# PatrykChrabaszcz/HpBandSter

Hardware: AMD Instinct MI355X
Metric: candidate KDE evals/sec (cand×obs pairs) at D=32, 1/2/4/8 MI355X; % VALU peak (higher is better)
Workload: dtype f16 MFMA coarse pre-screen (1 product per dim, rigorous bound), f32 accumulate, f64 re-score

## Files before the change

hpbandster_amd/csrc/hbx_acquire.h:

```cpp
#pragma once
#include "hbx_score.h"

struct KdePairRef {
  int32_t D;
  const void* params_good;
  const float* table_good;
  const double* X_good;
  const int64_t* rows_good;
  int32_t variant_good;
  const void* params_bad;
  const float* table_bad;
  const double* X_bad;
  const int64_t* rows_bad;
  int32_t variant_bad, dc_pad, du_pad;
  int64_t nmax;
  const KdeParams* Pg() const { return (const KdeParams*)params_good; }
  const KdeParams* Pb() const { return (const KdeParams*)params_bad; }
};

struct WsLayout {
  size_t res, U, count, flags, segcnt, segnear, best, key, first1, rescue, est_l, est_g, lo, list, near, exact_l,
      exact_g, part, total;
  size_t stage, seeds, surv, lpart;
  int32_t list_cap;
};
#define STAGED_LIST_CAP 4096
WsLayout ws_layout(int64_t Nc, int64_t nmax, int64_t B = 1);

struct AcqWs {
  AcqResult* res;
  uint32_t* U;
  int32_t *count, *flags, *segcnt, *segnear;
  uint64_t *best, *key;
  int32_t *first1, *rescue;
  KdeEst *el, *eg;
  float* lo;
  int32_t *list, *near;
  double *exact_l, *exact_g, *part;
  uint32_t* stage;
  int32_t *seeds, *surv;
  KdeEst* lpart;
  int32_t list_cap;
  AcqWs(void* workspace, const WsLayout& w) {
    char* ws = (char*)workspace;
    res = (AcqResult*)(ws + w.res);
    U = (uint32_t*)(ws + w.U);
    count = (int32_t*)(ws + w.count);
    flags = (int32_t*)(ws + w.flags);
    segcnt = (int32_t*)(ws + w.segcnt);
    segnear = (int32_t*)(ws + w.segnear);
    best = (uint64_t*)(ws + w.best);
    key = (uint64_t*)(ws + w.key);
    first1 = (int32_t*)(ws + w.first1);
    rescue = (int32_t*)(ws + w.rescue);
    el = (KdeEst*)(ws + w.est_l);
    eg = (KdeEst*)(ws + w.est_g);
    lo = (float*)(ws + w.lo);
    list = (int32_t*)(ws + w.list);
    near = (int32_t*)(ws + w.near);
    exact_l = (double*)(ws + w.exact_l);
    exact_g = (double*)(ws + w.exact_g);
    part = (double*)(ws + w.part);
    stage = (uint32_t*)(ws + w.stage);
    seeds = (int32_t*)(ws + w.seeds);
    surv = (int32_t*)(ws + w.surv);
    lpart = (KdeEst*)(ws + w.lpart);
    list_cap = w.list_cap;
  }
  KdePairArgs::AcqInitPtrs init() const { return {U, count, flags, first1, res}; }
};

struct AcqPlan {
  ScoreFns fg, fb;
  bool exact_only;
};
const KdePairRef* acq_pair(const char* who, const void* pair);
int acq_check(const char* who, const KdePairRef& p, const double* cand, int64_t Nc, const void* workspace);
int acq_plan(const KdePairRef& p, bool fast, AcqPlan* plan);
int acq_score(const AcqPlan& plan, const KdePairRef& p, const AcqWs& a, const ScoreRequest& rq, int64_t batch_B,
              ScoreResult* out);
#ifndef HBX_STAGED_MIN_PAIRS
#define HBX_STAGED_MIN_PAIRS 1e9
#endif
bool acq_staged_supported(const AcqPlan& plan);
int acq_score_staged(const AcqPlan& plan, const KdePairRef& p, const double* cand, int64_t Nc, const AcqWs& a,
                     hipEvent_t* ev, hipStream_t s);
int acq_exact_only_init(int64_t Nc, uint32_t seg, const AcqWs& a, hipStream_t s);
#define EXACT_SCAN_MAX 1024
int acq_exact(const KdePairRef& p, const double* cand, int64_t Nc, const AcqWs& a, bool scan, bool combine,
              hipStream_t s);
```

hpbandster_amd/csrc/hbx_common.h:

```cpp
#pragma once

#include <hip/hip_runtime.h>
#include <stdint.h>
#include <stdlib.h>

#define HBX_MAX_D 256
#define HBX_WAVE 64

#include "hbx.h"

int hbx_fail(int code, const char* fmt, ...);

#define HBX_HIP(call)                                                                 \
  do {                                                                                \
    hipError_t _e = (call);                                                           \
    if (_e != hipSuccess)                                                             \
      return hbx_fail(HBX_ERR_HIP, "%s failed: %s (%s:%d)", #call, hipGetErrorString(_e), \
                      __FILE__, __LINE__);                                            \
  } while (0)

#define HBX_LAUNCH_CHECK()                                                            \
  do {                                                                                \
    hipError_t _e = hipGetLastError();                                                \
    if (_e != hipSuccess)                                                             \
      return hbx_fail(HBX_ERR_HIP, "kernel launch failed: %s (%s:%d)",               \
                      hipGetErrorString(_e), __FILE__, __LINE__);                    \
  } while (0)

static inline bool hbx_switch_on(const char* name) {
  const char* e = getenv(name);
  return !(e && atoi(e) == 0);
}
static inline int hbx_staged_mode() {
  const char* e = getenv("HBX_STAGED");
  if (!e) return 1;
  const int v = atoi(e);
  return v == 0 ? 0 : v == 2 ? 2 : 1;
}

struct KdeParams {
  int32_t n;
  int32_t D;
  int32_t dc;
  int32_t du;
  int32_t nconst;
  int32_t nan_all;
  int32_t has_neg;
  int32_t unsupported;
  int32_t stride;
  int32_t dc_pad;
  int32_t du_pad;
  int32_t exact_only;
  double log_norm;
  double m0_log2;
  double lb_sum;
  double prod_bw_c;
  float cmax;
  float sum_abs_delta;
  float cmax2;
  int32_t pad1;
  int32_t kc;
  int32_t hmode;
  int32_t nsc;
  int32_t chunk_floats;
  int32_t oh_total;
  int32_t coarse_off;
  int32_t coarse_chunk_floats;
  const double* X;
  const int64_t* rows;
  int32_t oh_dim[64];
  int32_t oh_level[64];
  int32_t oh_col[64];
  double oh_val[64];
  int32_t oh_start[64];
  int32_t cat_maxcode[HBX_MAX_D];
  int32_t cont_dim[HBX_MAX_D];
  double cont_scale[HBX_MAX_D];
  double center[HBX_MAX_D];
  float xmax[HBX_MAX_D];
  int32_t cat_dim[HBX_MAX_D];
  float cat_delta[HBX_MAX_D];
  float cat_negf[HBX_MAX_D];
  int32_t const_dim[HBX_MAX_D];
  double const_level[HBX_MAX_D];
  int32_t vartype[HBX_MAX_D];
  int32_t nlev[HBX_MAX_D];
  double bw[HBX_MAX_D];
};

#define HBX_PARAM_STAGE ((sizeof(KdeParams) + 255) & ~(size_t)255)
#define HBX_COLSTATS_OFF (HBX_PARAM_STAGE + 8 * HBX_MAX_D + 4 * HBX_MAX_D + 64)
#define HBX_PARAM_BYTES (HBX_COLSTATS_OFF + 8 * HBX_MAX_D + 4 * HBX_MAX_D)
struct ColStats {
  double mean[HBX_MAX_D];
  int32_t maxcode[HBX_MAX_D];
};

struct KdeEst {
  float lpos;
  float lneg;
  float err;
  float pad;
};

struct AcqResult {
  int64_t index;
  double score;
  float rel;
  int32_t flags;
  int32_t shortlist;
  int32_t near;
  double pdf_l;
  double pdf_g;
};

__device__ __forceinline__ void hbx_publish_store(uint32_t* dst, uint32_t v) {
  __hip_atomic_store(dst, v, __ATOMIC_RELAXED, __HIP_MEMORY_SCOPE_SYSTEM);
}
__device__ __forceinline__ void hbx_publish_store64(uint64_t* dst, uint64_t v) {
  __hip_atomic_store(dst, v, __ATOMIC_RELAXED, __HIP_MEMORY_SCOPE_SYSTEM);
}
__device__ __forceinline__ void hbx_publish_done(int32_t* done, int32_t seq) {
  __asm__ volatile("s_waitcnt vmcnt(0)" ::: "memory");
  __hip_atomic_store(done, seq, __ATOMIC_RELAXED, __HIP_MEMORY_SCOPE_SYSTEM);
}

__device__ __forceinline__ uint32_t hbx_f2ord(float f) {
  uint32_t u = __float_as_uint(f);
  return (u & 0x80000000u) ? ~u : (u | 0x80000000u);
}
__device__ __forceinline__ float hbx_ord2f(uint32_t u) {
  return __uint_as_float((u & 0x80000000u) ? (u & 0x7fffffffu) : ~u);
}

__device__ __forceinline__ uint64_t hbx_d2ord(double d) {
  if (d != d) return ~0ull;
  if (d == 0.0) d = 0.0;
  uint64_t u = (uint64_t)__double_as_longlong(d);
  return (u & 0x8000000000000000ull) ? ~u : (u | 0x8000000000000000ull);
}

template <typename Op>
__device__ __forceinline__ uint32_t wave_reduce_dpp(uint32_t v, Op op) {
  v = op(v, (uint32_t)__builtin_amdgcn_update_dpp(0, (int)v, 0xb1, 0xf, 0xf, false));
  v = op(v, (uint32_t)__builtin_amdgcn_update_dpp(0, (int)v, 0x4e, 0xf, 0xf, false));
  v = op(v, (uint32_t)__builtin_amdgcn_update_dpp(0, (int)v, 0x141, 0xf, 0xf, false));
  v = op(v, (uint32_t)__builtin_amdgcn_update_dpp(0, (int)v, 0x140, 0xf, 0xf, false));
  return op(op((uint32_t)__builtin_amdgcn_readlane((int)v, 0), (uint32_t)__builtin_amdgcn_readlane((int)v, 16)),
            op((uint32_t)__builtin_amdgcn_readlane((int)v, 32), (uint32_t)__builtin_amdgcn_readlane((int)v, 48)));
}
struct OpAdd { __device__ uint32_t operator()(uint32_t a, uint32_t b) const { return a + b; } };
struct OpAnd { __device__ uint32_t operator()(uint32_t a, uint32_t b) const { return a & b; } };
struct OpOr { __device__ uint32_t operator()(uint32_t a, uint32_t b) const { return a | b; } };
struct OpMax { __device__ uint32_t operator()(uint32_t a, uint32_t b) const { return a > b ? a : b; } };
```

hpbandster_amd/csrc/hbx_kde.hip:

```cpp
#include "hbx_acquire.h"

#include <string.h>

#include <new>

#include "hbx_acq_impl.h"
#include "hbx_host.h"
#include "hbx_pairwise.h"
#include "hbx_rescue_impl.h"


__global__ void acq_init_kernel(uint32_t* U, int32_t* count, int32_t* flags, int32_t* first1, AcqResult* res) {
  if (threadIdx.x == 0 && blockIdx.x == 0) acq_init_state(U, count, flags, first1, res);
}

__global__ void acq_init_batch_kernel(int64_t B, uint32_t* __restrict__ U, int32_t* __restrict__ flags,
                                      int32_t* __restrict__ segcnt, uint64_t* __restrict__ best,
                                      uint64_t* __restrict__ key, int32_t* __restrict__ first1,
                                      int32_t* __restrict__ count, int32_t* __restrict__ segnear) {
  const int64_t b = (int64_t)blockIdx.x * blockDim.x + threadIdx.x;
  if (b == 0) *count = 0;
  if (b < B) {
    U[b] = hbx_f2ord(INFINITY);
    flags[b] = 0;
// ... 412 lines not shown
}

__global__ __launch_bounds__(256) void kde_exact_logs_kernel(const int32_t* __restrict__ list,
                                                             const int32_t* __restrict__ count,
                                                             const double* __restrict__ exact_l,
                                                             const double* __restrict__ exact_g,
                                                             float* __restrict__ logl, float* __restrict__ logg) {
  const int p = blockIdx.x * 256 + threadIdx.x;
  if (p >= *count) return;
  const int i = list[p];
  if (logl) logl[i] = (float)log(exact_l[p]);
  if (logg) logg[i] = (float)log(exact_g[p]);
}


WsLayout ws_layout(int64_t Nc, int64_t nmax, int64_t B) {
  WsLayout w;
  size_t o = 0;
  auto take = [&](size_t bytes) {
    size_t r = o;
    o += (bytes + 255) & ~(size_t)255;
    return r;
  };
  w.res = take(sizeof(AcqResult));
  w.count = take(4);
  w.U = take(4 * B);
  w.flags = take(4 * B);
  w.segcnt = take(4 * B);
  w.segnear = take(4 * B);
  w.best = take(8 * B);
  w.key = take(8 * B);
  w.first1 = take(4 * B);
  w.rescue = take(4);
  const int sp = obs_splits((unsigned)((Nc + 511) / 512), nmax, true);
  const int64_t cap16 = 16 * Nc < 196608 ? 16 * Nc : 196608;
  const int64_t nest = Nc * sp > cap16 ? Nc * sp : cap16;
  w.est_l = take(sizeof(KdeEst) * nest);
  w.est_g = take(sizeof(KdeEst) * nest);
  w.lo = take(4 * Nc);
  w.list = take(4 * Nc);
  w.near = take(4 * Nc);
  w.exact_l = take(8 * Nc);
  w.exact_g = take(8 * Nc);
  w.part = take(8 * (size_t)2 * EXACT_SPLIT_CAP * PW_SPLIT_UNITS * ((nmax + PW_BUF - 1) / PW_BUF));
  static_assert(sizeof(AcqResult) + 4 * HBX_ST_WORDS <= 256, "the state words fit the result slot's padding");
  w.stage = w.res + sizeof(AcqResult);
  const int64_t tiles = (Nc + 511) / 512;
  w.list_cap = (int32_t)(512 * (tiles < 1 ? 1 : tiles > STAGED_LIST_CAP / 512 ? STAGED_LIST_CAP / 512 : tiles));
  w.seeds = take(4 * (size_t)w.list_cap);
  w.surv = take(4 * Nc);
  w.lpart = take(sizeof(KdeEst) * (size_t)OBS_SPLIT_MAX * w.list_cap);
  w.total = o;
  return w;
}

int acq_check(const char* who, const KdePairRef& p, const double* cand, int64_t Nc, const void* workspace) {
  if ((!cand && Nc > 0) || !p.params_good || !p.table_good || !p.X_good || !p.rows_good || !p.params_bad ||
      !p.table_bad || !p.X_bad || !p.rows_bad || !workspace)
    return hbx_fail(HBX_ERR_ARG, "%s: null pointer", who);
  if (Nc < 0 || Nc > INT32_MAX) return hbx_fail(HBX_ERR_ARG, "Nc=%lld out of range", (long long)Nc);
  return HBX_OK;
}

const KdePairRef* acq_pair(const char* who, const void* pair) {
  if (!pair) hbx_fail(HBX_ERR_ARG, "%s: null pair", who);
  return (const KdePairRef*)pair;
}

int acq_plan(const KdePairRef& p, bool fast, AcqPlan* plan) {
  plan->exact_only = KdeVariant::decode(p.variant_good).exact_only || KdeVariant::decode(p.variant_bad).exact_only;
  plan->fg = pick_logpdf(p.dc_pad, p.du_pad, p.variant_good, fast);
  plan->fb = pick_logpdf(p.dc_pad, p.du_pad, p.variant_bad, fast);
  if (!plan->exact_only && (!plan->fg.main || !plan->fb.main))
    return hbx_fail(HBX_ERR_UNSUPPORTED, "no kernel for dc_pad=%d du_pad=%d", p.dc_pad, p.du_pad);
  return HBX_OK;
}

int acq_score(const AcqPlan& plan, const KdePairRef& p, const AcqWs& a, const ScoreRequest& rq, int64_t batch_B,
              ScoreResult* out) {
  *out = ScoreResult{};
  const hipStream_t s = rq.s;
  const bool scored = rq.Nc > 0 && !plan.exact_only;
  if (scored) {
    const int rc = launch_score2({plan.fg, p.params_good, p.table_good, a.el},
                                 {plan.fb, p.params_bad, p.table_bad, a.eg}, rq, out);
    if (rc) return rc;
  }
  if (batch_B) {
    hipLaunchKernelGGL(acq_init_batch_kernel, dim3((unsigned)((batch_B + 255) / 256)), dim3(256), 0, s, batch_B, a.U,
                       a.flags, a.segcnt, a.best, a.key, a.first1, a.count, a.segnear);
    HBX_LAUNCH_CHECK();
  } else if (!out->inited) {
    hipLaunchKernelGGL(acq_init_kernel, dim3(1), dim3(64), 0, s, a.U, a.count, a.flags, a.first1, a.res);
    HBX_LAUNCH_CHECK();
  }
  if (scored && (out->nsplit[0] > 1 || out->nsplit[1] > 1)) {
    hipLaunchKernelGGL(kde_merge_splits_kernel, dim3((unsigned)((2 * rq.Nc + 255) / 256)), dim3(256), 0, s, a.el,
                       a.eg, rq.Nc, out->nsplit[0], out->nsplit[1]);
    HBX_LAUNCH_CHECK();
  }
  return HBX_OK;
}

int acq_exact_only_init(int64_t Nc, uint32_t seg, const AcqWs& a, hipStream_t s) {
  hipLaunchKernelGGL(kde_exact_only_init_kernel, dim3((unsigned)((Nc + 255) / 256)), dim3(256), 0, s, Nc, seg, a.el,
                     a.eg, a.lo, a.flags);
  HBX_LAUNCH_CHECK();
  return HBX_OK;
}

struct AcqCall {
  const char* who;
  const double* cand;
  int64_t Nc, seg, index_base;
  float *logl_out, *logg_out;
  AcqResult* batch_res;
  void* workspace;
  int64_t ws_bytes;
  void *events, *stream;
  AcqResult* host_res;
  int32_t seq;
  PickOut pick;
};

static int acquire_impl(const void* pair, const AcqCall& c) {
  const KdePairRef* pp = acq_pair(c.who, pair);
  if (!pp) return HBX_ERR_ARG;
  const KdePairRef& p = *pp;
  const double* cand = c.cand;
  const int64_t Nc = c.Nc, seg = c.seg;
  float *logl_out = c.logl_out, *logg_out = c.logg_out;
  AcqResult* batch_res = c.batch_res;
  int rc = acq_check(c.who, p, cand, Nc, c.workspace);
  if (rc) return rc;
  if (seg < 1) return hbx_fail(HBX_ERR_ARG, "%s: segment length %lld", c.who, (long long)seg);
  const int64_t B = batch_res ? (Nc + seg - 1) / seg : 1;
  const WsLayout w = ws_layout(Nc, p.nmax, B);
  if ((size_t)c.ws_bytes < w.total)
    return hbx_fail(HBX_ERR_ARG, "workspace too small: %lld < %lld bytes", (long long)c.ws_bytes,
                    (long long)w.total);
  const bool fast = !logl_out && !logg_out;
  AcqPlan plan;
  rc = acq_plan(p, fast, &plan);
  if (rc) return rc;
  const AcqWs a(c.workspace, w);
  hipStream_t s = (hipStream_t)c.stream;
  hipEvent_t* ev = (hipEvent_t*)c.events;
  const uint32_t sg = (uint32_t)(batch_res ? seg : (Nc > 0 ? Nc : 1));
  if (B == 0) return HBX_OK;
  bool rescue_inline = false;
  const int stg = (!batch_res && fast && Nc > 0) ? hbx_staged_mode() : 0;
  const bool staged = stg && acq_staged_supported(plan) &&
                      (stg == 2 || (double)Nc * (double)p.nmax >= HBX_STAGED_MIN_PAIRS);
  if (staged) {
    rc = acq_score_staged(plan, p, cand, Nc, a, ev, s);
    rescue_inline = true;
  } else {
    const ScoreRequest rq{cand, Nc, p.D, ev, a.rescue, batch_res ? KdePairArgs::AcqInitPtrs{} : a.init(),
                          fast ? p.nmax : 0, !batch_res, s};
    ScoreResult sr;
    rc = acq_score(plan, p, a, rq, batch_res ? B : 0, &sr);
    rescue_inline = sr.rescue_inline;
  }
  if (rc) return rc;
  const dim3 grid((unsigned)((Nc + 255) / 256));
  bool fuse_combine = false;
  if (Nc > 0) {
    if (plan.exact_only) {
      rc = acq_exact_only_init(Nc, sg, a, s);
      if (rc) return rc;
    } else {
      const CombineRescue rs{cand, p.D, p.Pg(), p.Pb(), a.rescue};
      const bool sgn = KdeVariant::decode(p.variant_good).has_neg;
      const combine_fn cf = !rescue_inline ? kde_combine_kernel<false, false>
                            : sgn          ? kde_combine_kernel<true, true>
                                           : kde_combine_kernel<false, true>;
      hipLaunchKernelGGL(cf, dim3((unsigned)((Nc + 256 * COMBINE_SUB - 1) / (256 * COMBINE_SUB))), dim3(256), 0, s,
                         a.el, a.eg, Nc, sg, logl_out, logg_out, a.lo, a.U, a.flags, a.first1, rs);
      HBX_LAUNCH_CHECK();
    }
    const bool scan = !batch_res && Nc <= EXACT_SCAN_MAX;
    if (!scan) {
      hipLaunchKernelGGL(kde_shortlist_kernel, grid, dim3(256), 0, s, a.lo, Nc, sg, a.U, a.flags, a.list, a.count,
                         batch_res ? a.segcnt : (int32_t*)nullptr, a.first1, a.rescue);
      HBX_LAUNCH_CHECK();
    }
    fuse_combine = !batch_res && !(plan.exact_only && (logl_out || logg_out));
    rc = acq_exact(p, cand, Nc, a, scan, !fuse_combine, s);
    if (rc) return rc;
    if (plan.exact_only && (logl_out || logg_out)) {
      hipLaunchKernelGGL(kde_exact_logs_kernel, grid, dim3(256), 0, s, a.list, a.count, a.exact_l, a.exact_g, logl_out,
                         logg_out);
      HBX_LAUNCH_CHECK();
    }
  }
  if (!batch_res) {
    hipLaunchKernelGGL(kde_final_kernel, dim3(1), dim3(256), 0, s, a.list, a.count, a.exact_l, a.exact_g, a.flags,
                       c.index_base, p.Pg(), p.Pb(), a.el, a.eg, a.near, a.res,
                       (int32_t)((p.nmax + PW_BUF - 1) / PW_BUF), fuse_combine ? a.part : (const double*)nullptr,
                       a.exact_l, a.exact_g, c.host_res, c.seq, c.pick);
    HBX_LAUNCH_CHECK();
    return HBX_OK;
  }
  if (Nc > 0) {
    hipLaunchKernelGGL(kde_batch_min_kernel, grid, dim3(256), 0, s, a.list, a.count, sg, a.exact_l, a.exact_g, a.best);
    HBX_LAUNCH_CHECK();
    hipLaunchKernelGGL(kde_batch_key_kernel, grid, dim3(256), 0, s, a.list, a.count, sg, a.exact_l, a.exact_g, a.best,
                       a.key);
    HBX_LAUNCH_CHECK();
    hipLaunchKernelGGL(kde_batch_near_kernel, grid, dim3(256), 0, s, a.list, a.count, sg, a.exact_l, a.exact_g, a.key,
                       p.Pg(), p.Pb(), a.el, a.eg, a.near, a.segnear);
    HBX_LAUNCH_CHECK();
    hipLaunchKernelGGL(kde_batch_final_kernel, dim3((unsigned)((B + 255) / 256)), dim3(256), 0, s, B, a.key, a.segcnt,
                       a.flags, a.segnear, a.list, a.exact_l, a.exact_g, p.Pg(), p.Pb(), a.el, a.eg, c.index_base,
                       batch_res);
    HBX_LAUNCH_CHECK();
  }
  return HBX_OK;
}

extern "C" {

int64_t hbx_kde_workspace_bytes(int64_t Nc, int64_t nmax) { return (int64_t)ws_layout(Nc, nmax).total; }

int64_t hbx_kde_batch_workspace_bytes(int64_t Nc, int64_t seg, int64_t nmax) {
  if (seg < 1) return -1;
  return (int64_t)ws_layout(Nc, nmax, (Nc + seg - 1) / seg).total;
}

void* hbx_kde_result_ptr(void* workspace) { return (char*)workspace + ws_layout(0, 0).res; }

int hbx_kde_acquire(const double* cand, int64_t Nc, int64_t index_base, const void* pair, float* logl_out,
                    float* logg_out, void* workspace, int64_t ws_bytes, void* events, void* stream) {
  return acquire_impl(pair, {"hbx_kde_acquire", cand, Nc, Nc > 0 ? Nc : 1, index_base, logl_out, logg_out, nullptr,
                             workspace, ws_bytes, events, stream, nullptr, 0, PickOut{}});
}

int hbx_kde_acquire_batch(const double* cand, int64_t Nc, int64_t seg, int64_t index_base, const void* pair,
                          float* logl_out, float* logg_out, void* results, void* workspace, int64_t ws_bytes,
                          void* stream) {
  if (!results) return hbx_fail(HBX_ERR_ARG, "hbx_kde_acquire_batch: null results");
  return acquire_impl(pair, {"hbx_kde_acquire_batch", cand, Nc, seg, index_base, logl_out, logg_out,
                             (AcqResult*)results, workspace, ws_bytes, nullptr, stream, nullptr, 0, PickOut{}});
}

void* hbx_kde_pair_bind(int32_t D, const void* params_good, const float* table_good, const double* X_good,
                        const int64_t* rows_good, int32_t variant_good, const void* params_bad,
                        const float* table_bad, const double* X_bad, const int64_t* rows_bad, int32_t variant_bad,
                        int32_t dc_pad, int32_t du_pad, int64_t nmax) {
  if (D <= 0 || D > HBX_MAX_D || !params_good || !params_bad || nmax < 0) {
    hbx_fail(HBX_ERR_ARG, "hbx_kde_pair_bind: bad arguments (D=%d, nmax=%lld)", D, (long long)nmax);
    return nullptr;
  }
  KdePairRef* b = new (std::nothrow) KdePairRef{D, params_good, table_good, X_good, rows_good, variant_good,
                                                params_bad, table_bad, X_bad, rows_bad, variant_bad, dc_pad,
                                                du_pad, nmax};
  if (!b) hbx_fail(HBX_ERR_ARG, "hbx_kde_pair_bind: out of host memory");
  return b;
}

void hbx_kde_pair_free(void* pair) { delete (KdePairRef*)pair; }

int hbx_kde_acquire_bound(const void* pair, const double* cand, int64_t Nc, int64_t index_base, void* workspace,
                          int64_t ws_bytes, const uint8_t* err, void* events, void* stream, void* rec_out,
                          double* row_out) {
  const char* who = "hbx_kde_acquire_bound";
  if (!pair || !rec_out || Nc < 0) return hbx_fail(HBX_ERR_ARG, "hbx_kde_acquire_bound: bad arguments");
  const KdePairRef& b = *(const KdePairRef*)pair;
  MappedBuf* mb = nullptr;
  int rc = hbx_mapped_acq(&mb);
  if (rc) return rc;
  char* pub = mb->p + PUB_OFF;
  const int32_t seq = mb->seq;
  const hipStream_t s = (hipStream_t)stream;
  const bool pick = err || row_out;
  rc = acquire_impl(pair, {who, cand, Nc, Nc > 0 ? Nc : 1, index_base, nullptr, nullptr, nullptr, workspace, ws_bytes,
                           events, stream, pick ? nullptr : (AcqResult*)pub, seq,
                           pick ? PickOut{cand, err, Nc, b.D, pub} : PickOut{}});
  if (rc) return rc;
  constexpr int RW = (int)(sizeof(AcqResult) / 4);
  constexpr int64_t SPIN = 20000000;
  const volatile uint64_t* w = (const volatile uint64_t*)pub;
  uint32_t words[RW];
  rc = wait_tagged(w, RW, seq, words, s, SPIN, who);
  if (rc) return rc;
  AcqResult r;
  memcpy(&r, words, sizeof(AcqResult));
  if (pick) {
    uint32_t e = 0;
    rc = wait_tagged(w + RW, 1, seq, &e, s, SPIN, who);
    if (rc) return rc;
    if (e) r.flags |= HBX_ACQ_DOMAIN_ERR;
    if (row_out && r.index >= 0 && r.index - index_base < Nc) {
      rc = wait_tagged(w + RW + 1, 2 * b.D, seq, (uint32_t*)row_out, s, SPIN, who);
      if (rc) return rc;
    }
  }
  memcpy(rec_out, &r, sizeof(AcqResult));
  return HBX_OK;
}

int hbx_kde_ws_offsets(int64_t Nc, int64_t seg, int64_t nmax, int64_t* out) {
  if (!out || seg < 1) return hbx_fail(HBX_ERR_ARG, "hbx_kde_ws_offsets: bad arguments");
  const WsLayout w = ws_layout(Nc, nmax, seg >= Nc ? 1 : (Nc + seg - 1) / seg);
  out[0] = (int64_t)w.count;
  out[1] = (int64_t)w.list;
  out[2] = (int64_t)w.near;
  out[3] = (int64_t)w.exact_l;
  out[4] = (int64_t)w.exact_g;
  return HBX_OK;
}

}
```

hpbandster_amd/csrc/hbx_kde_impl.h:

```cpp
#pragma once
#include <math.h>
#include <stdlib.h>
#include <string.h>

#include <vector>

#include "hbx_common.h"

#define HBX_LN2f 0.69314718055994531f
#define HBX_LN_CLAMP (-18.420680743952367)
#define HBX_INV_SQRT_2PI 0.3989422804014327
#ifndef EXACT_GRID
#define EXACT_GRID 2048
#endif
#define SUM_BLOCK 32
#define OBS_CHUNK 64
#define KROW 80
#define MFMA_WAVES 8
#ifndef H_ROW_TILES
#define H_ROW_TILES 2
#endif
#ifndef H_WAVES_PER_EU
#if H_ROW_TILES <= 2
#define H_WAVES_PER_EU 4
// ... 43 lines not shown
  return 8 * (((h32_par(nsc, kp) + (sgn ? 16 * kp : 0) + 7) / 8) | 1);
}
__host__ __device__ constexpr int h32_chunk_floats(int nsc, int kp, int sgn = 0) {
  return (OBS_CHUNK * h32_ktp(nsc, kp, sgn) / 2 + 255) & ~255;
}
#define H32_ROW_MAX 112
__host__ __device__ constexpr int h32c_nd(int nsc) { return (6 + 8 * nsc + 15) / 16; }
__host__ __device__ constexpr int h32c_par(int nsc, int kp) { return (16 * h32c_nd(nsc) + 16 * kp + 2 * h32_ixw(kp) + 7) & ~7; }
__host__ __device__ constexpr int h32c_ktp(int nsc, int kp) { return 8 * (((h32c_par(nsc, kp) + 7) / 8) | 1); }
__host__ __device__ constexpr int h32c_chunk_floats(int nsc, int kp) {
  return (OBS_CHUNK * h32c_ktp(nsc, kp) / 2 + 255) & ~255;
}
struct KdeVariant {
  int has_neg;
  int kc;
  int hmode;
  int exact_only;
  int h32;
  int coarse;
  int small_codes;
  __host__ __device__ int encode() const {
    return has_neg | (kc << 1) | (hmode << 4) | (exact_only << 5) | (h32 << 6) | (coarse << 7) | (small_codes << 8);
  }
  __host__ __device__ static KdeVariant decode(int v) {
    return {v & 1, (v >> 1) & 7, (v >> 4) & 1, (v >> 5) & 1, (v >> 6) & 1, (v >> 7) & 1, (v >> 8) & 1};
  }
};


typedef float f32x4 __attribute__((ext_vector_type(4)));

__device__ __forceinline__ float cat_match(float a, float b) {
  const float d = a - b;
  return __builtin_amdgcn_fmed3f(fmaf(-d, d, 1.f), 0.f, 1.f);
}

__device__ __forceinline__ float cand_code(double xv) {
  return (xv == rint(xv) && fabs(xv) < 1e6) ? (float)xv : -1e9f;
}

__device__ __forceinline__ KdeEst finish_est_terms(const KdeParams* __restrict__ P, float S, float Sn, float off,
                                                   bool nan_c, float ci, float bnd, bool SIGNED, float sum_terms) {
  KdeEst o;
  o.pad = 0.f;
  if (nan_c || S != S) {
    o.lpos = NAN;
    o.lneg = -INFINITY;
    o.err = 0.f;
    return o;
  }
  const float lnorm = (float)P->log_norm;
  const float Sp = SIGNED ? (S - Sn) : S;
  o.lpos = (Sp > 0.f) ? (__log2f(Sp) + off) * HBX_LN2f + lnorm : -INFINITY;
  o.lneg = (SIGNED && Sn > 0.f) ? (__log2f(Sn) + off) * HBX_LN2f + lnorm : -INFINITY;
  const float u = 0x1p-24f;
  const float Mabs = fabsf(ci) + P->cmax + bnd + P->sum_abs_delta;
  const float dt = 3.f * (float)(P->dc + P->du + 4) * u * Mabs;
  const float es = sum_terms * u * (SIGNED ? 3.f : 1.f);
  o.err = 2.f * (dt * HBX_LN2f + es) + 16.f * u;
  return o;
}

__device__ __forceinline__ KdeEst finish_est(const KdeParams* __restrict__ P, float S, float Sn, float off,
                                             bool nan_c, float ci, float bnd, bool SIGNED, int chunk) {
  return finish_est_terms(P, S, Sn, off, nan_c, ci, bnd, SIGNED,
                          (float)chunk + (float)P->n / (float)chunk + 24.f);
}

__device__ __forceinline__ void stage_rows(const double* __restrict__ src, int64_t nv, int D, int DS, double* xs,
                                           int lane) {
  if (D <= 64) {
    const int rpp = 64 / D;
    const int lr = lane / D, lc = lane - lr * D;
    if (lr < rpp) {
      const int npf = (int)nv / rpp;
      const unsigned vo = (unsigned)(lr * D + lc), xo = (unsigned)(lr * DS + lc);
      const int sq = __builtin_amdgcn_readfirstlane(rpp * D), xq = __builtin_amdgcn_readfirstlane(rpp * DS);
      for (int p0 = 0; p0 < npf; p0 += 16) {
        double t[16];
#pragma unroll
        for (int q = 0; q < 16; ++q)
          if (p0 + q < npf) t[q] = (src + (int64_t)(p0 + q) * sq)[vo];
#pragma unroll
        for (int q = 0; q < 16; ++q)
          if (p0 + q < npf) (xs + (p0 + q) * xq)[xo] = t[q];
      }
      const int row = npf * rpp + lr;
      if (row < (int)nv) xs[row * DS + lc] = src[row * D + lc];
    }
    return;
  }
  const int tot = (int)nv * D;
  for (int e0 = 0; e0 < tot; e0 += 16 * 64) {
    double t[16];
    int at[16];
#pragma unroll
    for (int q = 0; q < 16; ++q) {
      const int e = min(e0 + 64 * q + lane, tot - 1);
      const int row = e / D;
      at[q] = row * DS + (e - row * D);
      t[q] = src[e];
    }
#pragma unroll
    for (int q = 0; q < 16; ++q) xs[at[q]] = t[q];
  }
}

typedef _Float16 f16x8 __attribute__((ext_vector_type(8)));
typedef _Float16 f16x16 __attribute__((ext_vector_type(16)));

typedef void (*logpdf_fn)(const double*, int64_t, int32_t, const KdeParams*, const float*, KdeEst*);

#ifndef HBX_PAIR_INIT
#define HBX_PAIR_INIT 1
#endif

struct KdePairArgs {
  const KdeParams* P0;
  const KdeParams* P1;
  const float* table0;
  const float* table1;
  KdeEst* out0;
  KdeEst* out1;
  unsigned nblk0;
  int32_t* rescue;
  struct AcqInitPtrs {
    uint32_t* U;
    int32_t* count;
    int32_t* flags;
    int32_t* first1;
    struct AcqResult* res;
  } init;
  unsigned tiles = 0;
  int32_t nsplit0 = 1, nsplit1 = 1;
  int32_t row_stage = 1;
};
typedef void (*logpdf_pair_fn)(const double*, int64_t, int32_t, KdePairArgs);
typedef void (*logpdf_co_fn)(const double*, int64_t, int32_t, const KdeParams*, const float*, KdeEst*, int32_t);

struct KdeListArgs {
  const KdeParams* P;
  const float* table;
  KdeEst* out;
  KdeEst* part;
  const int32_t* idx;
  const int32_t* count;
  int32_t* rescue;
  int32_t cap, maxcount, nsplit;
  unsigned tiles_cap;
  int32_t row_stage;
};
typedef void (*logpdf_list_fn)(const double*, int32_t, KdeListArgs);

enum { HBX_ST_FLAG = 0, HBX_ST_LMAX, HBX_ST_USEED, HBX_ST_NSEED, HBX_ST_NSURV, HBX_ST_WORDS };

__device__ __forceinline__ void acq_init_state(uint32_t* U, int32_t* count, int32_t* flags, int32_t* first1,
                                               AcqResult* res) {
  uint32_t* st = (uint32_t*)(res + 1);
  st[HBX_ST_FLAG] = 0;
  st[HBX_ST_LMAX] = hbx_f2ord(-INFINITY);
  st[HBX_ST_USEED] = hbx_f2ord(INFINITY);
  st[HBX_ST_NSEED] = 0;
  st[HBX_ST_NSURV] = 0;
  *U = hbx_f2ord(INFINITY);
  *first1 = INT32_MAX;
  *count = 0;
  *flags = 0;
  res->index = -1;
  res->score = NAN;
  res->pdf_l = NAN;
  res->pdf_g = NAN;
  res->shortlist = 0;
  res->flags = 0;
  res->near = 0;
  res->rel = 0.f;
}

__host__ __device__ inline KdeEst kde_est_neutral() {
  KdeEst e;
  e.lpos = -INFINITY;
  e.lneg = -INFINITY;
  e.err = 0.f;
  e.pad = 0.f;
  return e;
}

__host__ __device__ inline void obs_split_range(int nchunks, int r, int nsplit, int* c0, int* nch) {
  const int per = (nchunks + nsplit - 1) / nsplit;
  *c0 = r * per;
  const int e = (*c0 + per) < nchunks ? (*c0 + per) : nchunks;
  *nch = e - *c0;
}

struct RefitMeta {
  int64_t seg[2];
  int64_t n_good, n_bad;
  double fac_good, fac_bad;
  int32_t vt[HBX_MAX_D];
};
struct RefitMetaArgs {
  int64_t n, n_good, n_bad;
  double fac_good, fac_bad;
  int32_t D;
  uint32_t vt[HBX_MAX_D / 32];
};
#define REFIT_SORT_SMALL 1024
#define REFIT_INLINE 256
int refit_sort_small(double* X, double* loss, const double* staged, const double* staged_inline, int64_t n_new,
                     const RefitMetaArgs& a, RefitMeta* m, int64_t* order, int32_t* arrays, hipStream_t s);

int refit_fit_colstats(const double* X, int32_t D, const int64_t* seg_off, const int64_t* order, const int64_t* n_good,
                       const int64_t* n_bad, const double* fac_good, const double* fac_bad, const int32_t* vartype,
                       double* bw_good, double* bw_bad, int32_t* nlev_good, int32_t* nlev_bad, ColStats* cs_good,
                       ColStats* cs_bad, hipStream_t s);
#define FIT_TILE_ROWS 16384

logpdf_fn hbx_pick_f32(int dc_pad, int du_pad, bool sg);
logpdf_fn hbx_pick_oh(int dc_pad, int kc, bool sg);
logpdf_fn hbx_pick_h(int nsc, int kc, bool sg);
logpdf_pair_fn hbx_pick_h_pair(int nsc, int kc, bool sg);
logpdf_fn hbx_pick_h32(int nsc, int kp, bool sg, bool fast);
logpdf_co_fn hbx_pick_h32_co(int nsc, int kp);
logpdf_pair_fn hbx_pick_h32_pair(int nsc, int kp, bool sg, bool fast, bool coarse = false);
logpdf_pair_fn hbx_pick_h32_pair1(int nsc, int kp);
logpdf_list_fn hbx_pick_h32_list(int nsc, int kp);

int hbx_logpdf_estimate(const double* cand, int64_t Nc, int32_t D, const void* params, const float* table,
                        int32_t dc_pad, int32_t du_pad, int32_t variant, KdeEst* est, hipStream_t s);
int hbx_logpdf_exact_listed(const double* cand, int64_t Nc, int32_t D, const KdeParams* P, const double* X,
                            const int64_t* rows, double* out, const int32_t* list, const int32_t* count,
                            bool per_point, hipStream_t s);
```

hpbandster_amd/csrc/hbx_staged.hip:

```cpp
#include "hbx_acquire.h"

#include <hip/hip_ext.h>

#include "hbx_acq_impl.h"
#include "hbx_rescue_impl.h"

#define STAGED_PT 4
#define HBX_LN4f 1.3862943611198906f

__global__ __launch_bounds__(256) void staged_l_kernel(KdeEst* __restrict__ el, int64_t Nc, int32_t ns,
                                                       const double* __restrict__ cand, int32_t D,
                                                       const KdeParams* __restrict__ Pl,
                                                       const int32_t* __restrict__ rescue_cnt,
                                                       float* __restrict__ lhi, uint32_t* __restrict__ stage) {
  const int32_t nres = *rescue_cnt;
  KdeEst e[STAGED_PT];
  if (ns == 1) {
#pragma unroll
    for (int r = 0; r < STAGED_PT; ++r) {
      const int64_t i = ((int64_t)blockIdx.x * STAGED_PT + r) * 256 + threadIdx.x;
      if (i < Nc) e[r] = el[i];
    }
  }
  float best = -INFINITY;
#pragma unroll
  for (int r = 0; r < STAGED_PT; ++r) {
    const int64_t i = ((int64_t)blockIdx.x * STAGED_PT + r) * 256 + threadIdx.x;
    if (i >= Nc) continue;
    bool mark = false;
    if (ns > 1) {
      if (nres != 0)
        for (int q = 0; q < ns; ++q) mark = mark || el[(int64_t)q * Nc + i].err == -1.f;
      if (!mark) e[r] = merge_splits(el, Nc, i, ns);
    } else {
      mark = e[r].err == -1.f;
    }
    if (mark) e[r] = kde_rescue_one<0, false, true>(cand, i, D, Pl);
    if (ns > 1 || mark) el[i] = e[r];
    float lo, hi = NAN, pt;
    if (e[r].lpos == e[r].lpos) {
      est_interval(e[r], &lo, &hi, &pt);
      best = fmaxf(best, lo);
    }
    lhi[i] = hi;
  }
  __shared__ float rb[4];
  for (int o = 32; o > 0; o >>= 1) best = fmaxf(best, __shfl_xor(best, o));
  if ((threadIdx.x & 63) == 0) rb[threadIdx.x >> 6] = best;
  __syncthreads();
  if (threadIdx.x == 0) {
    const float b = fmaxf(fmaxf(rb[0], rb[1]), fmaxf(rb[2], rb[3]));
    const uint32_t o = hbx_f2ord(b);
    if (o > __hip_atomic_load(stage + HBX_ST_LMAX, __ATOMIC_RELAXED, __HIP_MEMORY_SCOPE_AGENT))
      atomicMax(stage + HBX_ST_LMAX, o);
  }
}

__device__ __forceinline__ int32_t staged_reserve(int n, int32_t* __restrict__ count) {
  __shared__ int32_t wtot[4];
  __shared__ int32_t base;
  const int lane = threadIdx.x & 63, wv = threadIdx.x >> 6;
  int incl = n;
  for (int o = 1; o < 64; o <<= 1) {
    const int t = __shfl_up(incl, o);
    if (lane >= o) incl += t;
  }
  if (lane == 63) wtot[wv] = incl;
  __syncthreads();
  int woff = 0, total = 0;
  for (int w = 0; w < 4; ++w) {
    if (w < wv) woff += wtot[w];
    total += wtot[w];
  }
  if (threadIdx.x == 0) base = total > 0 ? atomicAdd(count, total) : 0;
  __syncthreads();
  return base + woff + incl - n;
}

__global__ __launch_bounds__(256) void staged_seed_kernel(float* __restrict__ lhi, int64_t Nc,
                                                          KdeEst* __restrict__ eg, int32_t* __restrict__ seeds,
                                                          int32_t cap, uint32_t* __restrict__ stage) {
  const float thr = hbx_ord2f(stage[HBX_ST_LMAX]) - HBX_LN4f;
  bool f[STAGED_PT];
  int n = 0;
#pragma unroll
  for (int r = 0; r < STAGED_PT; ++r) {
    const int64_t i = ((int64_t)blockIdx.x * STAGED_PT + r) * 256 + threadIdx.x;
    f[r] = false;
    if (i < Nc) {
      const float h = lhi[i];
      f[r] = h == h && h >= thr;
    }
    n += f[r] ? 1 : 0;
  }
  int32_t off = staged_reserve(n, (int32_t*)stage + HBX_ST_NSEED);
  const KdeEst none = {0.f, -INFINITY, HBX_EST_NOT_EVAL, 0.f};
#pragma unroll
  for (int r = 0; r < STAGED_PT; ++r) {
    const int64_t i = ((int64_t)blockIdx.x * STAGED_PT + r) * 256 + threadIdx.x;
    if (i >= Nc) continue;
    bool seeded = false;
    if (f[r]) {
      if (off < cap) {
        seeds[off] = (int32_t)i;
        seeded = true;
      }
      ++off;
    }
    if (seeded) lhi[i] = NAN;
    else eg[i] = none;
  }
}

__global__ __launch_bounds__(256) void staged_merge_kernel(const KdeEst* __restrict__ part, int32_t cap, int32_t ns,
                                                           const int32_t* __restrict__ idx,
                                                           const int32_t* __restrict__ count, int32_t maxcount,
                                                           const KdeEst* __restrict__ el, KdeEst* __restrict__ eg,
                                                           const KdeParams* __restrict__ Pb,
                                                           uint32_t* __restrict__ stage, int32_t update_u) {
  int32_t cnt = *count;
  if (cnt > maxcount) cnt = maxcount;
  if (cnt > cap) return;
  const int32_t k = blockIdx.x * 256 + threadIdx.x;
  float h = INFINITY;
  if (k < cnt) {
    const int32_t i = idx[k];
    bool mark = false;
    for (int q = 0; q < ns; ++q) mark = mark || part[(int64_t)q * cap + k].err == -1.f;
    KdeEst e = {0.f, -INFINITY, -1.f, 0.f};
    if (!mark) e = merge_splits(part, cap, k, ns);
    eg[i] = e;
    if (update_u && !mark) {
      const ScoreIv v = score_interval(el[i], e);
      if (!v.lnan) h = v.shi;
    }
  }
  if (update_u) {
    const bool guard = Pb->log_norm + log((double)(Pb->n > 1 ? Pb->n : 1)) < 600.0;
    for (int o = 32; o > 0; o >>= 1) h = fminf(h, __shfl_xor(h, o));
    if ((threadIdx.x & 63) == 0 && guard && h < INFINITY) {
      const uint32_t o = hbx_f2ord(h);
      if (o < __hip_atomic_load(stage + HBX_ST_USEED, __ATOMIC_RELAXED, __HIP_MEMORY_SCOPE_AGENT))
        atomicMin(stage + HBX_ST_USEED, o);
    }
  }
}

__global__ __launch_bounds__(256) void staged_survivor_kernel(const float* __restrict__ lhi, int64_t Nc,
                                                              int32_t* __restrict__ surv,
                                                              uint32_t* __restrict__ stage) {
  const float U = hbx_ord2f(stage[HBX_ST_USEED]);
  const float C = (float)HBX_LN_CLAMP;
  bool f[STAGED_PT];
  int n = 0;
#pragma unroll
  for (int r = 0; r < STAGED_PT; ++r) {
    const int64_t i = ((int64_t)blockIdx.x * STAGED_PT + r) * 256 + threadIdx.x;
    f[r] = false;
    if (i < Nc) {
      const float h = lhi[i];
      f[r] = h == h && (C - fmaxf(h, C)) <= U;
    }
    n += f[r] ? 1 : 0;
  }
  int32_t off = staged_reserve(n, (int32_t*)stage + HBX_ST_NSURV);
#pragma unroll
  for (int r = 0; r < STAGED_PT; ++r) {
    const int64_t i = ((int64_t)blockIdx.x * STAGED_PT + r) * 256 + threadIdx.x;
    if (i < Nc && f[r]) surv[off++] = (int32_t)i;
  }
  if (blockIdx.x == 0 && threadIdx.x == 0) stage[HBX_ST_FLAG] = 1;
}


bool acq_staged_supported(const AcqPlan& plan) {
  return HBX_PAIR_INIT && !plan.exact_only && plan.fg.list && plan.fb.list && plan.fg.pair && plan.fg.split_ok;
}

int acq_score_staged(const AcqPlan& plan, const KdePairRef& p, const double* cand, int64_t Nc, const AcqWs& a,
                     hipEvent_t* ev, hipStream_t s) {
  const ScoreFns& f = plan.fg;
  const PairShape sh = pair_shape(f, true, 1, Nc, p.nmax);
  const int ns = sh.nsplit;
  const unsigned grid = sh.tiles * (unsigned)ns;
  KdePairArgs ka{p.Pg(), p.Pg(), p.table_good, p.table_good, a.el, a.el, grid, a.rescue, a.init()};
  ka.tiles = sh.tiles;
  ka.nsplit0 = ka.nsplit1 = ns;
  ka.row_stage = hbx_row_stage();
  if (ev)
    hipExtLaunchKernelGGL(sh.kernel, dim3(grid), dim3(f.threads), 0, s, ev[0], nullptr, 0, cand, Nc, p.D, ka);
  else
    hipLaunchKernelGGL(sh.kernel, dim3(grid), dim3(f.threads), 0, s, cand, Nc, p.D, ka);
  HBX_LAUNCH_CHECK();
  const dim3 gsel((unsigned)((Nc + 256 * STAGED_PT - 1) / (256 * STAGED_PT)));
  hipLaunchKernelGGL(staged_l_kernel, gsel, dim3(256), 0, s, a.el, Nc, (int32_t)ns, cand, p.D, p.Pg(), a.rescue, a.lo,
                     a.stage);
  HBX_LAUNCH_CHECK();
  const int32_t cap = a.list_cap;
  hipLaunchKernelGGL(staged_seed_kernel, gsel, dim3(256), 0, s, a.lo, Nc, a.eg, a.seeds, cap, a.stage);
  HBX_LAUNCH_CHECK();
  const ScoreFns& fb = plan.fb;
  const int ls = list_splits(p.nmax);
  const unsigned tcap = (unsigned)(cap / fb.cands_per_block);
  KdeListArgs la{p.Pb(), p.table_bad, a.eg, a.lpart, a.seeds, (const int32_t*)a.stage + HBX_ST_NSEED, a.rescue, cap,
                 cap, ls, tcap, ka.row_stage};
  hipLaunchKernelGGL(fb.list, dim3(tcap * (unsigned)ls), dim3(fb.threads), 0, s, cand, p.D, la);
  HBX_LAUNCH_CHECK();
  const dim3 gmerge((unsigned)((cap + 255) / 256));
  hipLaunchKernelGGL(staged_merge_kernel, gmerge, dim3(256), 0, s, a.lpart, cap, (int32_t)ls, a.seeds, la.count, cap,
                     a.el, a.eg, p.Pb(), a.stage, 1);
  HBX_LAUNCH_CHECK();
  hipLaunchKernelGGL(staged_survivor_kernel, gsel, dim3(256), 0, s, a.lo, Nc, a.surv, a.stage);
  HBX_LAUNCH_CHECK();
  la.idx = a.surv;
  la.count = (const int32_t*)a.stage + HBX_ST_NSURV;
  la.maxcount = (int32_t)Nc;
  const unsigned gfull = (unsigned)((Nc + fb.cands_per_block - 1) / fb.cands_per_block);
  const unsigned gsplit = tcap * (unsigned)ls;
  hipLaunchKernelGGL(fb.list, dim3(gfull > gsplit ? gfull : gsplit), dim3(fb.threads), 0, s, cand, p.D, la);
  HBX_LAUNCH_CHECK();
  hipLaunchKernelGGL(staged_merge_kernel, gmerge, dim3(256), 0, s, a.lpart, cap, (int32_t)ls, a.surv, la.count,
                     (int32_t)Nc, a.el, a.eg, p.Pb(), a.stage, 0);
  HBX_LAUNCH_CHECK();
  if (ev) {
    HBX_HIP(hipEventRecord(ev[1], s));
    HBX_HIP(hipEventRecord(ev[2], s));
  }
  return HBX_OK;
}

extern "C" {

int hbx_kde_acquire_stats(const void* workspace, int64_t Nc, int64_t nmax, int64_t* out) {
  if (!workspace || !out || Nc < 0) return hbx_fail(HBX_ERR_ARG, "hbx_kde_acquire_stats: bad arguments");
  const WsLayout w = ws_layout(Nc, nmax);
  uint32_t st[HBX_ST_WORDS];
  HBX_HIP(hipDeviceSynchronize());
  HBX_HIP(hipMemcpy(st, (const char*)workspace + w.stage, sizeof(st), hipMemcpyDeviceToHost));
  const bool staged = st[HBX_ST_FLAG] == 1;
  const int64_t seeds = staged ? ((int64_t)st[HBX_ST_NSEED] < w.list_cap ? (int64_t)st[HBX_ST_NSEED] : w.list_cap) : 0;
  const int64_t surv = staged ? (int64_t)st[HBX_ST_NSURV] : 0;
  out[0] = staged ? 1 : 0;
  out[1] = seeds;
  out[2] = surv;
  out[3] = staged ? seeds + surv : Nc;
  return HBX_OK;
}

}
```

Baseline: 29980 billion.

## Fuse staged merge, combine and shortlist into compacted tail kernels

Adds a tail path to the staged acquisition pipeline. Instead of running the final merge, a full-Nc combine kernel and a full-Nc shortlist kernel, it runs a fused tail kernel that only touches seeded and surviving candidates. That kernel merges splits, rescues, computes score intervals, updates the bound atomically and compacts a pre-shortlist, followed by a single-block shortlist pass. The survivor kernel also writes the low bounds for non-survivors and skips the redundant eg writes. This is meant to remove full-array passes and kernel launches, but it relies on a single-block shortlist and on correct handling of the overflow case (full scan).

```diff
diff --git a/hpbandster_amd/csrc/hbx_acquire.h b/hpbandster_amd/csrc/hbx_acquire.h
--- a/hpbandster_amd/csrc/hbx_acquire.h
+++ b/hpbandster_amd/csrc/hbx_acquire.h
@@ -84,7 +84,7 @@
 #endif
 bool acq_staged_supported(const AcqPlan& plan);
 int acq_score_staged(const AcqPlan& plan, const KdePairRef& p, const double* cand, int64_t Nc, const AcqWs& a,
-                     hipEvent_t* ev, hipStream_t s);
+                     hipEvent_t* ev, hipStream_t s, bool tail);
 int acq_exact_only_init(int64_t Nc, uint32_t seg, const AcqWs& a, hipStream_t s);
 #define EXACT_SCAN_MAX 1024
 int acq_exact(const KdePairRef& p, const double* cand, int64_t Nc, const AcqWs& a, bool scan, bool combine,
diff --git a/hpbandster_amd/csrc/hbx_common.h b/hpbandster_amd/csrc/hbx_common.h
--- a/hpbandster_amd/csrc/hbx_common.h
+++ b/hpbandster_amd/csrc/hbx_common.h
@@ -37,6 +37,7 @@
   const int v = atoi(e);
   return v == 0 ? 0 : v == 2 ? 2 : 1;
 }
+static inline bool hbx_staged_tail() { return hbx_switch_on("HBX_STAGED_TAIL"); }
 
 struct KdeParams {
   int32_t n;
diff --git a/hpbandster_amd/csrc/hbx_kde.hip b/hpbandster_amd/csrc/hbx_kde.hip
--- a/hpbandster_amd/csrc/hbx_kde.hip
+++ b/hpbandster_amd/csrc/hbx_kde.hip
@@ -588,8 +588,9 @@
   const int stg = (!batch_res && fast && Nc > 0) ? hbx_staged_mode() : 0;
   const bool staged = stg && acq_staged_supported(plan) &&
                       (stg == 2 || (double)Nc * (double)p.nmax >= HBX_STAGED_MIN_PAIRS);
+  const bool tail = staged && hbx_staged_tail();
   if (staged) {
-    rc = acq_score_staged(plan, p, cand, Nc, a, ev, s);
+    rc = acq_score_staged(plan, p, cand, Nc, a, ev, s, tail);
     rescue_inline = true;
   } else {
     const ScoreRequest rq{cand, Nc, p.D, ev, a.rescue, batch_res ? KdePairArgs::AcqInitPtrs{} : a.init(),
@@ -605,7 +606,7 @@
     if (plan.exact_only) {
       rc = acq_exact_only_init(Nc, sg, a, s);
       if (rc) return rc;
-    } else {
+    } else if (!tail) {
       const CombineRescue rs{cand, p.D, p.Pg(), p.Pb(), a.rescue};
       const bool sgn = KdeVariant::decode(p.variant_good).has_neg;
       const combine_fn cf = !rescue_inline ? kde_combine_kernel<false, false>
@@ -615,8 +616,8 @@
                          a.el, a.eg, Nc, sg, logl_out, logg_out, a.lo, a.U, a.flags, a.first1, rs);
       HBX_LAUNCH_CHECK();
     }
-    const bool scan = !batch_res && Nc <= EXACT_SCAN_MAX;
-    if (!scan) {
+    const bool scan = !batch_res && Nc <= EXACT_SCAN_MAX && !tail;
+    if (!scan && !tail) {
       hipLaunchKernelGGL(kde_shortlist_kernel, grid, dim3(256), 0, s, a.lo, Nc, sg, a.U, a.flags, a.list, a.count,
                          batch_res ? a.segcnt : (int32_t*)nullptr, a.first1, a.rescue);
       HBX_LAUNCH_CHECK();
diff --git a/hpbandster_amd/csrc/hbx_kde_impl.h b/hpbandster_amd/csrc/hbx_kde_impl.h
--- a/hpbandster_amd/csrc/hbx_kde_impl.h
+++ b/hpbandster_amd/csrc/hbx_kde_impl.h
@@ -219,7 +219,15 @@
 };
 typedef void (*logpdf_list_fn)(const double*, int32_t, KdeListArgs);
 
-enum { HBX_ST_FLAG = 0, HBX_ST_LMAX, HBX_ST_USEED, HBX_ST_NSEED, HBX_ST_NSURV, HBX_ST_WORDS };
+enum {
+  HBX_ST_FLAG = 0,
+  HBX_ST_LMAX,
+  HBX_ST_USEED,
+  HBX_ST_NSEED,
+  HBX_ST_NSURV,
+  HBX_ST_NPRE,
+  HBX_ST_WORDS
+};
 
 __device__ __forceinline__ void acq_init_state(uint32_t* U, int32_t* count, int32_t* flags, int32_t* first1,
                                                AcqResult* res) {
@@ -229,6 +237,7 @@
   st[HBX_ST_USEED] = hbx_f2ord(INFINITY);
   st[HBX_ST_NSEED] = 0;
   st[HBX_ST_NSURV] = 0;
+  st[HBX_ST_NPRE] = 0;
   *U = hbx_f2ord(INFINITY);
   *first1 = INT32_MAX;
   *count = 0;
diff --git a/hpbandster_amd/csrc/hbx_staged.hip b/hpbandster_amd/csrc/hbx_staged.hip
--- a/hpbandster_amd/csrc/hbx_staged.hip
+++ b/hpbandster_amd/csrc/hbx_staged.hip
@@ -79,7 +79,8 @@
 
 __global__ __launch_bounds__(256) void staged_seed_kernel(float* __restrict__ lhi, int64_t Nc,
                                                           KdeEst* __restrict__ eg, int32_t* __restrict__ seeds,
-                                                          int32_t cap, uint32_t* __restrict__ stage) {
+                                                          int32_t cap, uint32_t* __restrict__ stage,
+                                                          int32_t mark_rest) {
   const float thr = hbx_ord2f(stage[HBX_ST_LMAX]) - HBX_LN4f;
   bool f[STAGED_PT];
   int n = 0;
@@ -108,7 +109,7 @@
       ++off;
     }
     if (seeded) lhi[i] = NAN;
-    else eg[i] = none;
+    else if (mark_rest) eg[i] = none;
   }
 }
 
@@ -146,9 +147,10 @@
   }
 }
 
-__global__ __launch_bounds__(256) void staged_survivor_kernel(const float* __restrict__ lhi, int64_t Nc,
+__global__ __launch_bounds__(256) void staged_survivor_kernel(float* __restrict__ lhi, int64_t Nc,
                                                               int32_t* __restrict__ surv,
-                                                              uint32_t* __restrict__ stage) {
+                                                              uint32_t* __restrict__ stage,
+                                                              int32_t* __restrict__ flags) {
   const float U = hbx_ord2f(stage[HBX_ST_USEED]);
   const float C = (float)HBX_LN_CLAMP;
   bool f[STAGED_PT];
@@ -160,6 +162,10 @@
     if (i < Nc) {
       const float h = lhi[i];
       f[r] = h == h && (C - fmaxf(h, C)) <= U;
+      if (flags && h == h) {
+        lhi[i] = C - fmaxf(h, C);
+        if (h > 700.f) atomicOr(flags, 1);
+      }
     }
     n += f[r] ? 1 : 0;
   }
@@ -172,13 +178,203 @@
   if (blockIdx.x == 0 && threadIdx.x == 0) stage[HBX_ST_FLAG] = 1;
 }
 
+struct StagedTailArgs {
+  const KdeEst* part;
+  int32_t cap, ns;
+  const int32_t* seeds;
+  const int32_t* surv;
+  int64_t Nc;
+  const double* cand;
+  int32_t D;
+  const KdeParams* Pb;
+  const KdeEst* el;
+  KdeEst* eg;
+  float* lo;
+  uint32_t* U;
+  int32_t* flags;
+  int32_t* first1;
+  int32_t* list;
+  int32_t* count;
+  int32_t* rescue_cnt;
+  uint32_t* stage;
+};
+
+__device__ __forceinline__ uint32_t ld_agent(const uint32_t* p) {
+  return __hip_atomic_load(p, __ATOMIC_RELAXED, __HIP_MEMORY_SCOPE_AGENT);
+}
+__device__ __forceinline__ int32_t ld_agent(const int32_t* p) {
+  return __hip_atomic_load(p, __ATOMIC_RELAXED, __HIP_MEMORY_SCOPE_AGENT);
+}
+
+#define TAIL_THREADS 1024
+#define TAIL_PT 4
+__global__ __launch_bounds__(256) void staged_tail_kernel(StagedTailArgs t) {
+  constexpr int TAIL_THREADS_A = 256;
+  constexpr int NW = TAIL_THREADS_A / 64;
+  __shared__ int32_t swc[NW];
+  __shared__ uint32_t pbase;
+  const int lane = threadIdx.x & 63, wv = threadIdx.x >> 6;
+  int64_t nseed = (int32_t)t.stage[HBX_ST_NSEED], nsurv = (int32_t)t.stage[HBX_ST_NSURV];
+  if (nseed > t.cap) nseed = t.cap;
+  if (nsurv > t.Nc) nsurv = t.Nc;
+  const bool split = nsurv <= t.cap;
+  const int64_t total = nseed + nsurv;
+  constexpr int64_t EPB = (int64_t)TAIL_PT * TAIL_THREADS_A;
+  const int64_t nwork = (total + EPB - 1) / EPB;
+  if (blockIdx.x >= nwork) return;
+  const int32_t nres = *t.rescue_cnt;
+  int32_t idx[TAIL_PT];
+  KdeEst ea[TAIL_PT], eb[TAIL_PT];
+  float slo[TAIL_PT];
+#pragma unroll
+  for (int r = 0; r < TAIL_PT; ++r) {
+    const int64_t k = (int64_t)blockIdx.x * EPB + r * TAIL_THREADS_A + threadIdx.x;
+    idx[r] = -1;
+    if (k < total) idx[r] = k < nseed ? t.seeds[k] : t.surv[k - nseed];
+  }
+#pragma unroll
+  for (int r = 0; r < TAIL_PT; ++r) {
+    const int64_t k = (int64_t)blockIdx.x * EPB + r * TAIL_THREADS_A + threadIdx.x;
+    if (idx[r] < 0) continue;
+    ea[r] = t.el[idx[r]];
+    if (k < nseed || !split) eb[r] = t.eg[idx[r]];
+  }
+  float h = INFINITY;
+  int32_t f1 = INT32_MAX;
+  bool of = false;
+#pragma unroll
+  for (int r = 0; r < TAIL_PT; ++r) {
+    const int64_t k = (int64_t)blockIdx.x * EPB + r * TAIL_THREADS_A + threadIdx.x;
+    slo[r] = NAN;
+    if (idx[r] < 0) continue;
+    const int64_t i = idx[r];
+    bool store = false;
+    if (!(k < nseed || !split)) {
+      const int64_t ks = k - nseed;
+      bool mark = false;
+      for (int q = 0; q < t.ns; ++q) mark = mark || t.part[(int64_t)q * t.cap + ks].err == -1.f;
+      eb[r] = {0.f, -INFINITY, -1.f, 0.f};
+      if (!mark) eb[r] = merge_splits(t.part, t.cap, ks, t.ns);
+      store = true;
+    }
+    if (nres != 0 && eb[r].err == -1.f) {
+      eb[r] = kde_rescue_one<0, false, true>(t.cand, i, t.D, t.Pb);
+      store = true;
+    }
+    if (store) t.eg[i] = eb[r];
+    const ScoreIv v = score_interval(ea[r], eb[r]);
+    slo[r] = v.one ? NAN : v.slo;
+    t.lo[i] = slo[r];
+    if (!v.lnan) h = fminf(h, v.shi);
+    if (v.one && (int32_t)i < f1) f1 = (int32_t)i;
+    of = of || v.of;
+  }
+  float hw = h;
+  int32_t fw = f1;
+  for (int o = 32; o > 0; o >>= 1) {
+    hw = fminf(hw, __shfl_xor(hw, o));
+    fw = min(fw, __shfl_xor(fw, o));
+  }
+  const bool ofw = __ballot(of) != 0;
+  bool lowered = false;
+  if (lane == 0) {
+    const uint32_t o = hbx_f2ord(hw);
+    if (hw < INFINITY && o < ld_agent(t.U)) atomicMin(t.U, o);
+    if (fw != INT32_MAX && fw < ld_agent(t.first1)) lowered = atomicMin(t.first1, fw) > fw;
+    if (ofw) atomicOr(t.flags, 1);
+  }
+  lowered = __shfl(lowered ? 1 : 0, 0) != 0;
+  __syncthreads();
+  const float useed = hbx_ord2f(t.stage[HBX_ST_USEED]);
+  const float u = fminf(useed, hbx_ord2f(ld_agent(t.U)));
+  int n = 0;
+#pragma unroll
+  for (int r = 0; r < TAIL_PT; ++r) {
+    const float l = slo[r];
+    if (!(idx[r] >= 0 && ((l == l && l <= u) || (lowered && idx[r] == fw)))) idx[r] = -1;
+    n += idx[r] >= 0 ? 1 : 0;
+  }
+  {
+    int incl = n;
+    for (int o = 1; o < 64; o <<= 1) {
+      const int v = __shfl_up(incl, o);
+      if (lane >= o) incl += v;
+    }
+    if (lane == 63) swc[wv] = incl;
+    __syncthreads();
+    int off = incl - n, tot = 0;
+#pragma unroll
+    for (int w = 0; w < NW; ++w) {
+      off += w < wv ? swc[w] : 0;
+      tot += swc[w];
+    }
+    if (threadIdx.x == 0) pbase = tot > 0 ? atomicAdd(t.stage + HBX_ST_NPRE, (uint32_t)tot) : 0u;
+    __syncthreads();
+    off += (int)pbase;
+#pragma unroll
+    for (int r = 0; r < TAIL_PT; ++r)
+      if (idx[r] >= 0) t.list[off++] = idx[r];
+  }
+}
+
+__global__ __launch_bounds__(TAIL_THREADS) void staged_shortlist_kernel(StagedTailArgs t) {
+  constexpr int NW = TAIL_THREADS / 64;
+  constexpr int64_t EPB = (int64_t)TAIL_PT * TAIL_THREADS;
+  __shared__ int32_t swc[NW];
+  const int lane = threadIdx.x & 63, wv = threadIdx.x >> 6;
+  const int64_t npre = t.stage[HBX_ST_NPRE];
+  const float uf = hbx_ord2f(t.U[0]);
+  const int32_t ff = t.first1[0];
+  const bool all = (t.flags[0] & 1) != 0;
+  const int64_t nscan = all ? t.Nc : npre;
+  int64_t base = 0;
+  for (int64_t c0 = 0; c0 < nscan; c0 += EPB) {
+    const int64_t c = c0 + (int64_t)TAIL_PT * threadIdx.x;
+    int32_t ci[TAIL_PT];
+    float cl[TAIL_PT];
+#pragma unroll
+    for (int r = 0; r < TAIL_PT; ++r) ci[r] = c + r < nscan ? (all ? (int32_t)(c + r) : t.list[c + r]) : -1;
+#pragma unroll
+    for (int r = 0; r < TAIL_PT; ++r) cl[r] = ci[r] >= 0 ? t.lo[ci[r]] : NAN;
+    int n = 0;
+#pragma unroll
+    for (int r = 0; r < TAIL_PT; ++r) {
+      if (!(ci[r] >= 0 && ((cl[r] == cl[r] && (all || cl[r] <= uf)) || ci[r] == ff))) ci[r] = -1;
+      n += ci[r] >= 0 ? 1 : 0;
+    }
+    int incl = n;
+    for (int o = 1; o < 64; o <<= 1) {
+      const int v = __shfl_up(incl, o);
+      if (lane >= o) incl += v;
+    }
+    if (lane == 63) swc[wv] = incl;
+    __syncthreads();
+    int64_t off = base + incl - n;
+    int tot = 0;
+#pragma unroll
+    for (int w = 0; w < NW; ++w) {
+      off += w < wv ? swc[w] : 0;
+      tot += swc[w];
+    }
+#pragma unroll
+    for (int r = 0; r < TAIL_PT; ++r)
+      if (ci[r] >= 0) t.list[off++] = ci[r];
+    base += tot;
+    __syncthreads();
+  }
+  if (threadIdx.x == 0) {
+    *t.count = (int32_t)base;
+    *t.rescue_cnt = 0;
+  }
+}
+
 
 bool acq_staged_supported(const AcqPlan& plan) {
   return HBX_PAIR_INIT && !plan.exact_only && plan.fg.list && plan.fb.list && plan.fg.pair && plan.fg.split_ok;
 }
 
 int acq_score_staged(const AcqPlan& plan, const KdePairRef& p, const double* cand, int64_t Nc, const AcqWs& a,
-                     hipEvent_t* ev, hipStream_t s) {
+                     hipEvent_t* ev, hipStream_t s, bool tail) {
   const ScoreFns& f = plan.fg;
   const PairShape sh = pair_shape(f, true, 1, Nc, p.nmax);
   const int ns = sh.nsplit;
@@ -197,7 +393,8 @@
                      a.stage);
   HBX_LAUNCH_CHECK();
   const int32_t cap = a.list_cap;
-  hipLaunchKernelGGL(staged_seed_kernel, gsel, dim3(256), 0, s, a.lo, Nc, a.eg, a.seeds, cap, a.stage);
+  hipLaunchKernelGGL(staged_seed_kernel, gsel, dim3(256), 0, s, a.lo, Nc, a.eg, a.seeds, cap, a.stage,
+                     (int32_t)(tail ? 0 : 1));
   HBX_LAUNCH_CHECK();
   const ScoreFns& fb = plan.fb;
   const int ls = list_splits(p.nmax);
@@ -210,7 +407,8 @@
   hipLaunchKernelGGL(staged_merge_kernel, gmerge, dim3(256), 0, s, a.lpart, cap, (int32_t)ls, a.seeds, la.count, cap,
                      a.el, a.eg, p.Pb(), a.stage, 1);
   HBX_LAUNCH_CHECK();
-  hipLaunchKernelGGL(staged_survivor_kernel, gsel, dim3(256), 0, s, a.lo, Nc, a.surv, a.stage);
+  hipLaunchKernelGGL(staged_survivor_kernel, gsel, dim3(256), 0, s, a.lo, Nc, a.surv, a.stage,
+                     tail ? a.flags : (int32_t*)nullptr);
   HBX_LAUNCH_CHECK();
   la.idx = a.surv;
   la.count = (const int32_t*)a.stage + HBX_ST_NSURV;
@@ -219,8 +417,17 @@
   const unsigned gsplit = tcap * (unsigned)ls;
   hipLaunchKernelGGL(fb.list, dim3(gfull > gsplit ? gfull : gsplit), dim3(fb.threads), 0, s, cand, p.D, la);
   HBX_LAUNCH_CHECK();
-  hipLaunchKernelGGL(staged_merge_kernel, gmerge, dim3(256), 0, s, a.lpart, cap, (int32_t)ls, a.surv, la.count,
-                     (int32_t)Nc, a.el, a.eg, p.Pb(), a.stage, 0);
+  if (tail) {
+    const StagedTailArgs ta{a.lpart, cap,     (int32_t)ls, a.seeds,  a.surv, Nc,      cand,     p.D,      p.Pb(),
+                            a.el,    a.eg,    a.lo,        a.U,      a.flags, a.first1, a.list, a.count, a.rescue,
+                            a.stage};
+    hipLaunchKernelGGL(staged_tail_kernel, dim3((unsigned)((Nc + cap + 1023) / 1024)), dim3(256), 0, s, ta);
+    HBX_LAUNCH_CHECK();
+    hipLaunchKernelGGL(staged_shortlist_kernel, dim3(1), dim3(TAIL_THREADS), 0, s, ta);
+  } else {
+    hipLaunchKernelGGL(staged_merge_kernel, gmerge, dim3(256), 0, s, a.lpart, cap, (int32_t)ls, a.surv, la.count,
+                       (int32_t)Nc, a.el, a.eg, p.Pb(), a.stage, 0);
+  }
   HBX_LAUNCH_CHECK();
   if (ev) {
     HBX_HIP(hipEventRecord(ev[1], s));
```

Measured after the change: 30620 billion, median of 6. 2.1% higher.
